# sbyrnes321/metalens

Hardware: AMD Instinct MI355X
Metric: aperture x far-field pair-evals/sec (higher is better)
Workload: dtype f64; 1 GPU; 1 mm dia NA=0.5 lens, lambda=580 nm, 4096x4096 aperture window at pitch lambda/2.2 -> 512x512 far-field directions (bins of the aperture FFT lattice x 1), fp64, on-axis x-dipole at the focus; aperture=4096, farfield=512, rings=197, centre_cells=1219855, orders=survey, pmc_key=gpus=1,aperture=4096,farfield=512,precision=f64,method=auto,zoom=1,pols=1, pmc_stale=True

## Files before the change

metalens_amd/csrc/zfft.hip:

```cpp
#include <cmath>
#include <cstdlib>
#include <map>
#include <tuple>
#include <utility>

#include "common.h"
#include "zfft_core.h"

namespace ml {

using zf::cd;

struct FftArgs {
    zf::Geo g;
    const cd *in;
    int64_t in_s1, in_s2, in_es;
    int in_rb;
    int a0, h0, a1, h1;
    const int *row_first;
    int rf_mod;
    int sub_s, sub_i;
    cd *out;
    int64_t out_s1, out_s2, out_es;
    int out_rb;
    const cd *tw1;
    const cd *wk;
    const cd *pj;
    const int *kbin;
    double alpha[4];
    int alpha_rb;
    int rows, chunk, accumulate;
};

template <int R3T>
__device__ __forceinline__ zf::Geo geo_of(const FftArgs &a) {
    zf::Geo g = a.g;
    if (R3T > 0) g.R3 = R3T;
    return g;
}

template <int R3T, bool STREAM>
__device__ __forceinline__ void load_row(const FftArgs &a, const zf::Geo &g, int row, int tid, cd *v) {
    const int NT = 16 * g.R3;
    const cd *src = a.in + (row / a.in_rb) * a.in_s1 + (row % a.in_rb) * a.in_s2;
    const int first = a.row_first ? a.row_first[row % a.rf_mod] : 0;
#pragma unroll
    for (int n2 = 0; n2 < 16; ++n2) {
        const int n = (tid + NT * n2) * a.sub_s + a.sub_i;
        int q = -1;
        if (n >= a.a0 && n < a.a0 + a.h0) q = n - a.a0;
        if (n >= a.a1 && n < a.a1 + a.h1) q = a.h0 + n - a.a1;
        if (min(n, g.n_valid - 1 - n) < first) q = -1;
        if (STREAM && q >= 0) {
            typedef double double2v __attribute__((ext_vector_type(2)));
            const double2v t = __builtin_nontemporal_load(reinterpret_cast<const double2v *>(src + q * a.in_es));
            v[n2] = zf::mk(t.x, t.y);
        } else {
            v[n2] = q >= 0 ? src[q * a.in_es] : zf::mk(0.0, 0.0);
        }
    }
}

template <int PASS>
__device__ __forceinline__ int64_t out_off(const FftArgs &a, int j) {
    return PASS == 4 ? zf::tile_off(j, a.out_es) : (int64_t)j * a.out_es;
}

__device__ __forceinline__ int row_of_turn(const FftArgs &a, int xcd, int idx) {
    const int row = xcd * a.chunk + idx;
    return idx < a.chunk && row < a.rows ? row : -1;
}

template <int R3T, int NTMAX, int MINW, int PASS, bool IP>
__global__ __launch_bounds__(NTMAX, MINW) void zfft_kernel(const FftArgs a) {
    extern __shared__ __align__(16) unsigned char zfft_lds_raw[];
    cd *lds = reinterpret_cast<cd *>(zfft_lds_raw);
    const zf::Geo g = geo_of<R3T>(a);
    const int NT = 16 * g.R3, tid = threadIdx.x;
    cd *s_tw = lds + zf::lds_elems(g);
    for (int e = tid; e < 256; e += NT) s_tw[(e & 15) * 16 + (e >> 4)] = a.tw1[e];
    const int n1 = tid / g.R3;
    cd tb[4];
    tb[0] = zf::mk(1.0, 0.0);
#pragma unroll
    for (int b = 1; b < 4; ++b) tb[b] = a.tw1[n1 * 16 + b];
    const int bin0 = tid, bin1 = tid + NT;
    const bool own0 = bin0 < g.M, own1 = bin1 < g.M, few = g.M <= 2 * NT;
    cd w0 = zf::mk(0, 0), p0 = w0, w1 = w0, p1 = w0;
    int k0 = 0, k1 = 0;
    if (own0) {
        w0 = a.wk[bin0];
        p0 = a.pj[bin0];
        k0 = a.kbin[bin0];
    }
    if (own1) {
        w1 = a.wk[bin1];
        p1 = a.pj[bin1];
        k1 = a.kbin[bin1];
    }
    const bool pair = own0 && own1 && ((k1 - k0) & 255) == 0;
    __syncthreads();
    const int xcd = blockIdx.x & 7, step = gridDim.x >> 3;
    int idx = blockIdx.x >> 3;
    int row = row_of_turn(a, xcd, idx);
    cd v[16], nx[16];
    if (row >= 0) load_row<R3T, PASS != 2>(a, g, row, tid, v);
    while (row >= 0) {
        const int idx_n = idx + step, row_n = row_of_turn(a, xcd, idx_n);
        const bool more = row_n >= 0;
        if (more) load_row<R3T, PASS != 2>(a, g, row_n, tid, nx);
        {
            cd ta[4];
            ta[0] = tb[0];
#pragma unroll
            for (int q = 1; q < 4; ++q) ta[q] = s_tw[(4 * q) * 16 + n1];
            zf::stage1_regs(g, tid, v, ta, tb, lds);
        }
        __syncthreads();
        zf::gather2(g, tid, v, lds);
        if (IP) {
            zf::scatter2_ip(g, tid, v, lds);
        } else {
            __syncthreads();
            zf::scatter2(g, tid, v, lds);
        }
        __syncthreads();
        cd *dst = a.out + (row / a.out_rb) * a.out_s1 + (row % a.out_rb) * a.out_s2;
        const double al = a.alpha[row / a.alpha_rb];
        if (few && pair) {
            cd xa, xb;
            if (IP)
                zf::stage3_pair_ip(g, k0, w0, w1, lds, xa, xb);
            else
                zf::stage3_pair(g, k0, w0, w1, lds, xa, xb);
            xa = zf::cmul(xa, p0);
            xb = zf::cmul(xb, p1);
            xa.x *= al;
            xa.y *= al;
            xb.x *= al;
            xb.y *= al;
            cd *da = dst + out_off<PASS>(a, bin0), *db = dst + out_off<PASS>(a, bin1);
            if (a.accumulate) {
                xa = zf::cadd(xa, *da);
                xb = zf::cadd(xb, *db);
            }
            *da = xa;
            *db = xb;
        } else if (few) {
            if (own0) {
                cd x = zf::cmul(IP ? zf::stage3_ip(g, k0, w0, lds) : zf::stage3(g, k0, w0, lds), p0);
                x.x *= al;
                x.y *= al;
                cd *d = dst + out_off<PASS>(a, bin0);
                if (a.accumulate) x = zf::cadd(x, *d);
                *d = x;
            }
            if (own1) {
                cd x = zf::cmul(IP ? zf::stage3_ip(g, k1, w1, lds) : zf::stage3(g, k1, w1, lds), p1);
                x.x *= al;
                x.y *= al;
                cd *d = dst + out_off<PASS>(a, bin1);
                if (a.accumulate) x = zf::cadd(x, *d);
                *d = x;
            }
        } else {
            for (int o = tid; o < g.M; o += NT) {
                const cd w = a.wk[o], p = a.pj[o];
                cd x = zf::cmul(IP ? zf::stage3_ip(g, a.kbin[o], w, lds) : zf::stage3(g, a.kbin[o], w, lds), p);
                x.x *= al;
                x.y *= al;
                cd *d = dst + out_off<PASS>(a, o);
                if (a.accumulate) x = zf::cadd(x, *d);
                *d = x;
            }
        }
        __syncthreads();
#pragma unroll
        for (int n2 = 0; n2 < 16; ++n2) v[n2] = nx[n2];
        idx = idx_n;
        row = row_n;
    }
}

template <int A, bool STREAM>
__device__ __forceinline__ void load_row_mixed(const FftArgs &a, const zf::Geo &g, int row, int tid, int stride, cd *v) {
    const cd *src = a.in + (row / a.in_rb) * a.in_s1 + (row % a.in_rb) * a.in_s2;
    const int first = a.row_first ? a.row_first[row % a.rf_mod] : 0;
#pragma unroll
    for (int n2 = 0; n2 < A; ++n2) {
        const int n = tid + stride * n2;
        int q = -1;
        if (n >= a.a0 && n < a.a0 + a.h0) q = n - a.a0;
        if (n >= a.a1 && n < a.a1 + a.h1) q = a.h0 + n - a.a1;
        if (min(n, g.n_valid - 1 - n) < first) q = -1;
        if (STREAM && q >= 0) {
            typedef double double2v __attribute__((ext_vector_type(2)));
            const double2v t = __builtin_nontemporal_load(reinterpret_cast<const double2v *>(src + q * a.in_es));
            v[n2] = zf::mk(t.x, t.y);
        } else {
            v[n2] = q >= 0 ? src[q * a.in_es] : zf::mk(0.0, 0.0);
        }
    }
}

template <int A, int B, bool STREAM>
__global__ __launch_bounds__(512) void zfft_mixed_kernel(const FftArgs a) {
    extern __shared__ __align__(16) unsigned char zfft_lds_raw[];
    cd *lds = reinterpret_cast<cd *>(zfft_lds_raw);
    const zf::Geo g = a.g;
    constexpr int LMAX = A > B ? A : B;
    const int R = g.R3, NT = LMAX * R, tid = threadIdx.x;
    cd *s_tw = lds + zf::mx_lds_elems<A, B>(g);
    for (int e = tid; e < A * B; e += NT) s_tw[(e % A) * B + e / A] = a.tw1[e];
    const bool act1 = tid < B * R, act2 = tid < A * R;
    __syncthreads();
    const int xcd = blockIdx.x & 7, step = gridDim.x >> 3;
    int idx = blockIdx.x >> 3;
    int row = row_of_turn(a, xcd, idx);
    cd v[LMAX], nx[A];
    if (row >= 0 && act1) load_row_mixed<A, STREAM>(a, g, row, tid, B * R, v);
    while (row >= 0) {
        const int idx_n = idx + step, row_n = row_of_turn(a, xcd, idx_n);
        if (row_n >= 0 && act1) load_row_mixed<A, STREAM>(a, g, row_n, tid, B * R, nx);
        if (act1) zf::mx_stage1<A, B>(g, tid, v, s_tw, lds);
        __syncthreads();
        if (act2) zf::mx_stage2<A, B>(g, tid, v, lds);
        __syncthreads();
        cd *dst = a.out + (row / a.out_rb) * a.out_s1 + (row % a.out_rb) * a.out_s2;
        const double al = a.alpha[row / a.alpha_rb];
        for (int o = tid; o < g.M; o += NT) {
            cd x = zf::cmul(zf::mx_stage3<A, B>(g, a.kbin[o], a.wk[o], lds), a.pj[o]);
            x.x *= al;
            x.y *= al;
            cd *d = dst + (int64_t)o * a.out_es;
            if (a.accumulate) x = zf::cadd(x, *d);
            *d = x;
        }
        __syncthreads();
#pragma unroll
        for (int n2 = 0; n2 < A; ++n2) v[n2] = nx[n2];
        idx = idx_n;
        row = row_n;
    }
}

template <int A, int B, bool STREAM>
static int launch_mixed(hipStream_t stream, const FftArgs &a, int threads, int grid, size_t lds_bytes) {
    auto kern = zfft_mixed_kernel<A, B, STREAM>;
    static bool attr_done = false;
    if (!attr_done) {
        ML_HIP(hipFuncSetAttribute(reinterpret_cast<const void *>(kern),
                                   hipFuncAttributeMaxDynamicSharedMemorySize, 160 * 1024));
        attr_done = true;
    }
    hipLaunchKernelGGL(kern, dim3(grid), dim3(threads), lds_bytes, stream, a);
    ML_HIP(hipGetLastError());
    return ML_OK;
}

__device__ __forceinline__ void load_tile(const FftArgs &a, const cd *src, int n0, int m1, cd *v) {
#pragma unroll
    for (int m2 = 0; m2 < 16; ++m2) {
        const int n = n0 + a.g.R3 * (m1 + 16 * m2);
        int q = -1;
        if (n0 >= 0 && n >= a.a0 && n < a.a0 + a.h0) q = n - a.a0;
        if (n0 >= 0 && n >= a.a1 && n < a.a1 + a.h1) q = a.h0 + n - a.a1;
        if (q >= 0) {
            typedef double double2v __attribute__((ext_vector_type(2)));
// ... 127 lines not shown
#pragma unroll
            for (int q = 0; q < (PAIR ? NB / 2 : NB); ++q) {
                const int oa = tid + NT * q, ob = oa + 256;
                if (PAIR) {
                    if (ob < gp.M) {
                        const cd wa = a.wk[oa], wb = a.wk[ob];
                        cd xa, xb;
                        zf::stage3_pair(gp, kq[q], wa, wb, lds, xa, xb);
                        if (p == P - 1) {
                            acc[q] = xa;
                            acc[q + NB / 2] = xb;
                        } else {
                            acc[q] = zf::cmac(acc[q], s_wr[oa], xa);
                            acc[q + NB / 2] = zf::cmac(acc[q + NB / 2], s_wr[ob], xb);
                        }
                        continue;
                    }
                }
                if (oa < gp.M) {
                    const cd wa = a.wk[oa];
                    const cd xa = zf::stage3(gp, kq[q], wa, lds);
                    if (p == P - 1) {
                        acc[q] = xa;
                    } else {
                        acc[q] = zf::cmac(acc[q], s_wr[oa], xa);
                    }
                }
                if (PAIR) acc[q + NB / 2] = zf::mk(0.0, 0.0);
            }
            __syncthreads();
        }
        cd *dst = a.out + (row / a.out_rb) * a.out_s1 + (row % a.out_rb) * a.out_s2;
        const double al = a.alpha[row / a.alpha_rb];
#pragma unroll
        for (int q = 0; q < NB; ++q) {
            const int o = tid + NT * q;
            if (o < gp.M) {
                cd x = zf::cmul(acc[q], a.pj[o]);
                x.x *= al;
                x.y *= al;
                cd *d = dst + o * a.out_es;
                if (a.accumulate) x = zf::cadd(x, *d);
                *d = x;
            }
        }
        idx = idx_n;
        row = row_n;
    }
}

template <int R3P, int P, int NB, int MINW, int PASS>
static int launch_pass(hipStream_t stream, const FftArgs &a, int grid, size_t lds_bytes) {
    auto kern = zfft_pass_kernel<R3P, P, NB, MINW, PASS>;
    static bool attr_done = false;
    if (!attr_done) {
        ML_HIP(hipFuncSetAttribute(reinterpret_cast<const void *>(kern),
                                   hipFuncAttributeMaxDynamicSharedMemorySize, 160 * 1024));
        attr_done = true;
    }
    hipLaunchKernelGGL(kern, dim3(grid), dim3(16 * R3P), lds_bytes, stream, a);
    ML_HIP(hipGetLastError());
    return ML_OK;
}

template <int PASS>
__global__ __launch_bounds__(256) void zfft_multi_kernel(const FftArgs a, int cpw) {
    extern __shared__ __align__(16) unsigned char zfft_lds_raw[];
    const zf::Geo g = a.g;
    const int NT = 16 * g.R3, sub = threadIdx.x / NT, tid = threadIdx.x - sub * NT;
    cd *lds = reinterpret_cast<cd *>(zfft_lds_raw) + (size_t)sub * zf::lds_elems(g);
    cd *s_tw = reinterpret_cast<cd *>(zfft_lds_raw) + (size_t)cpw * zf::lds_elems(g);
    for (int e = threadIdx.x; e < 256; e += blockDim.x) s_tw[(e & 15) * 16 + (e >> 4)] = a.tw1[e];
    const int n1 = tid / g.R3;
    __syncthreads();
    const int groups = (a.rows + cpw - 1) / cpw, chunk = (groups + 7) / 8;
    const int xcd = blockIdx.x & 7, step = gridDim.x >> 3;
    for (int idx = blockIdx.x >> 3; idx < chunk; idx += step) {
        const int grp = xcd * chunk + idx;
        if (grp >= groups) break;
        const int row = grp * cpw + sub;
        const bool live = row < a.rows;
        cd v[16];
        if (live) {
            load_row<0, PASS != 2>(a, g, row, tid, v);
        } else {
#pragma unroll
            for (int n2 = 0; n2 < 16; ++n2) v[n2] = zf::mk(0.0, 0.0);
        }
        zf::stage1_inplace(g, tid, v, s_tw, n1, lds);
        __syncthreads();
        zf::gather2(g, tid, v, lds);
        __syncthreads();
        zf::scatter2(g, tid, v, lds);
        __syncthreads();
        if (live) {
            cd *dst = a.out + (row / a.out_rb) * a.out_s1 + (row % a.out_rb) * a.out_s2;
            const double al = a.alpha[row / a.alpha_rb];
            for (int o = tid; o < g.M; o += NT) {
                cd x = zf::cmul(zf::stage3(g, a.kbin[o], a.wk[o], lds), a.pj[o]);
                x.x *= al;
                x.y *= al;
                cd *d = dst + o * a.out_es;
                if (a.accumulate) x = zf::cadd(x, *d);
                *d = x;
            }
        }
        __syncthreads();
    }
}

__global__ __launch_bounds__(512) void zfft_interleaved_kernel(const FftArgs a, int s, int64_t sub_off, int stuff) {
    extern __shared__ __align__(16) unsigned char zfft_lds_raw[];
    const zf::Geo g = a.g;
    const int NT = 16 * g.R3, sub = threadIdx.x / NT, tid = threadIdx.x - sub * NT, T = NT * s;
    cd *base = reinterpret_cast<cd *>(zfft_lds_raw);
    const int stride = zf::lds_elems(g);
    cd *lds = base + (size_t)sub * stride;
    cd *s_tw = base + (size_t)s * stride;
    for (int e = threadIdx.x; e < 256; e += T) s_tw[(e & 15) * 16 + (e >> 4)] = a.tw1[e];
    const int n1 = tid / g.R3;
    __syncthreads();
    const int chunk = (a.rows + 7) / 8, xcd = blockIdx.x & 7, step = gridDim.x >> 3;
    for (int idx = blockIdx.x >> 3; idx < chunk; idx += step) {
        const int row = xcd * chunk + idx;
        if (row >= a.rows) break;
        const cd *src = a.in + (row / a.in_rb) * a.in_s1 + (row % a.in_rb) * a.in_s2 + sub * sub_off;
        cd v[16];
#pragma unroll
        for (int n2 = 0; n2 < 16; ++n2) {
            const int n = tid + NT * n2, m = n / stuff;
            const int lrow = m * s + sub;
            v[n2] = (m * stuff == n && m < g.n_valid && lrow >= a.a0 && lrow < a.a0 + a.h0) ? src[(int64_t)m * a.in_es]
                                                                                             : zf::mk(0.0, 0.0);
        }
        zf::stage1_inplace(g, tid, v, s_tw, n1, lds);
        __syncthreads();
        zf::gather2(g, tid, v, lds);
        __syncthreads();
        zf::scatter2(g, tid, v, lds);
        __syncthreads();
        cd *dst = a.out + (row / a.out_rb) * a.out_s1 + (row % a.out_rb) * a.out_s2;
        const double al = a.alpha[row / a.alpha_rb];
        for (int o = threadIdx.x; o < g.M; o += T) {
            const int k = a.kbin[o];
            const cd w = a.wk[o];
            cd x = zf::mk(0.0, 0.0);
            for (int i = 0; i < s; ++i)
                x = zf::cmac(zf::stage3(g, k, w, base + (size_t)i * stride), a.pj[(size_t)i * g.M + o], x);
            x.x *= al;
            x.y *= al;
            cd *d = dst + o * a.out_es;
            if (a.accumulate) x = zf::cadd(x, *d);
            *d = x;
        }
        __syncthreads();
    }
}

constexpr int C128_PITCH = 9;
__global__ __launch_bounds__(64) void zfft_cols128_kernel(const FftArgs a, int64_t sub_off) {
    __shared__ cd s_a[8 * 16 * C128_PITCH];
    __shared__ cd s_tw[8 * 16];
    const int lane = threadIdx.x, i = lane >> 3, t = lane & 7;
    for (int e = lane; e < 128; e += 64) s_tw[e] = a.tw1[(2 * (e >> 4)) * 16 + (e & 15)];
    const int M = a.g.M, n_have = a.g.n_valid;
    const int chunk = (a.rows + 7) / 8, xcd = blockIdx.x & 7, step = gridDim.x >> 3;
    for (int idx = blockIdx.x >> 3; idx < chunk; idx += step) {
// ... 243 lines not shown
    }
    const int tiles = c.rows / 8, grid = std::min(tiles, 256);
    hipLaunchKernelGGL(zfft_tiles_kernel, dim3(grid), dim3(L.threads), bytes, stream, a);
    ML_HIP(hipGetLastError());
    return ML_OK;
}

static int zfft_run_mixed(hipStream_t stream, const ZfftCall &c) {
    FftArgs a = args_of(c);
    const int A = c.mixA, B = c.mixB, R = c.N_eff / (A * B), threads = std::max(A, B) * R;
    ML_REQUIRE(A * B * R == c.N_eff && R >= 1 && R <= 32 && threads <= 512 && c.sub_s <= 1 && !c.tiled_out &&
                   c.passes <= 1 && c.pad1 >= 0 && c.pad1 <= 16,
               "mixed-radix transform: %d samples as %d x %d x %d", c.N_eff, A, B, R);
    a.g.R3 = R;
    a.g.pad2 = 0;
    const size_t lds_bytes = ((size_t)(B * R + c.pad1) * A + A * B) * sizeof(cd);
    ML_REQUIRE(lds_bytes <= 160 * 1024, "mixed-radix transform: %d samples do not fit one workgroup", c.N_eff);
    const int per_cu = (int)std::min<size_t>({(size_t)8, std::max<size_t>(1, (160 * 1024) / lds_bytes),
                                              (size_t)std::max(1, 1024 / ((threads + 63) / 64 * 64))});
    int grid = std::min(256 * per_cu, a.chunk * 8);
    grid = (grid + 7) / 8 * 8;
#define ML_MIXED(AA, BB)                                                                            \
    if (A == AA && B == BB)                                                                         \
        return c.in_es == 1 ? launch_mixed<AA, BB, true>(stream, a, threads, grid, lds_bytes)       \
                            : launch_mixed<AA, BB, false>(stream, a, threads, grid, lds_bytes);
    ZF_MX_PAIRS(ML_MIXED)
#undef ML_MIXED
    set_error("mixed-radix transform: no kernel for legs %d x %d", A, B);
    return ML_EINVAL;
}

int zfft_run(hipStream_t stream, const ZfftCall &c) {
    if (c.mixA) return zfft_run_mixed(stream, c);
    FftArgs a = args_of(c);
    ML_REQUIRE(!c.tiled_out || (a.g.R3 >= 3 && a.g.R3 <= 16 && c.passes <= 1 && c.in_es == 1 && !c.second),
               "tiled row pass: %d samples", c.N_eff);
    ZfftLaunchFacts f;
    f.N_eff = c.N_eff, f.M = c.M, f.passes = c.passes;
    f.contiguous = c.in_es == 1, f.second = c.second != 0, f.tiled_out = c.tiled_out != 0;
    const ZfftLaunch L = zfft_launch_rule(f);
    if (L.family == ZfftFamily::multi) {
        const int cpw = L.cpw;
        const size_t bytes = ((size_t)cpw * zf::lds_elems(a.g) + 256) * sizeof(cd);
        const int groups = (a.rows + cpw - 1) / cpw;
        int grid = std::min(256 * 8, (groups + 7) / 8 * 8);
        grid = std::max(grid, 8);
        if (L.PASS == 1)
            hipLaunchKernelGGL(zfft_multi_kernel<1>, dim3(grid), dim3(L.threads), bytes, stream, a, cpw);
        else
            hipLaunchKernelGGL(zfft_multi_kernel<2>, dim3(grid), dim3(L.threads), bytes, stream, a, cpw);
        ML_HIP(hipGetLastError());
        return ML_OK;
    }
    size_t lds_bytes = ((size_t)zf::lds_elems(a.g) + 256) * sizeof(cd);
    const int per_cu = (int)std::min<size_t>(8, std::max<size_t>(1, (160 * 1024) / lds_bytes));
    int grid = std::min(256 * per_cu, a.chunk * 8);
    grid = (grid + 7) / 8 * 8;
    if (L.family == ZfftFamily::pass) {
        const int P = L.P, M = a.g.M;
        FftArgs ap = a;
        zfft_choose_pads(c.N_eff / P, M, c.j0, &ap.g.pad1, &ap.g.pad2, c.jstep);
        zf::Geo gp = ap.g;
        gp.R3 = L.R3P;
        const size_t bytes = ((size_t)zf::lds_elems(gp) + 256 + M) * sizeof(cd);
        const int per = (int)std::min<size_t>(8, std::max<size_t>(1, (160 * 1024) / bytes));
        int gridp = std::min(256 * per, a.chunk * 8);
        gridp = (gridp + 7) / 8 * 8;
#define ML_PASS(R, PP, NBB)                                                                          \
    if (L.R3P == R && L.P == PP && L.NB == NBB)                                                      \
        return L.PASS == 3   ? launch_pass<R, PP, NBB, 2, 3>(stream, ap, gridp, bytes)               \
               : L.PASS == 1 ? launch_pass<R, PP, NBB, 2, 1>(stream, ap, gridp, bytes)               \
                             : launch_pass<R, PP, NBB, 2, 2>(stream, ap, gridp, bytes);
        ML_PASS(16, 2, 2)
        ML_PASS(32, 2, 2)
#undef ML_PASS
    }
    ML_REQUIRE(L.family == ZfftFamily::one, "a lattice of %d samples does not fit one workgroup (%d wanted bins)",
               c.N_eff, c.M);
    if (L.ip) {
        a.g.ip = 1;
        zfft_choose_pads(-c.N_eff, c.M, c.j0, &a.g.pad1, &a.g.pad2, c.jstep);
        lds_bytes = ((size_t)zf::lds_elems(a.g) + 256) * sizeof(cd);
    }
    if (L.PASS == 3) switch (L.R3T) {
            case 8: return launch_one<8, 128, 2, 3>(stream, a, grid, lds_bytes);
            case 16: return launch_one<16, 256, 2, 3>(stream, a, grid, lds_bytes);
            default: return launch_one<32, 512, 2, 3>(stream, a, grid, lds_bytes);
        }
    if (L.PASS == 4) switch (L.R3T) {
            case 4: return launch_one<4, 64, 2, 4>(stream, a, grid, lds_bytes);
            case 8: return launch_one<8, 128, 2, 4>(stream, a, grid, lds_bytes);
            case 16: return launch_one<16, 256, 2, 4>(stream, a, grid, lds_bytes);
            default: return launch_one<0, 512, 1, 4>(stream, a, grid, lds_bytes);
        }
    if (L.PASS == 1) switch (L.R3T) {
            case 4: return launch_one<4, 64, 2, 1>(stream, a, grid, lds_bytes);
            case 8: return launch_one<8, 128, 2, 1>(stream, a, grid, lds_bytes);
            case 16: return launch_one<16, 256, 2, 1>(stream, a, grid, lds_bytes);
            case 32: return launch_one<32, 512, 2, 1>(stream, a, grid, lds_bytes);
            default: return launch_one<0, 512, 1, 1>(stream, a, grid, lds_bytes);
        }
    switch (L.R3T) {
        case 4: return launch_one<4, 64, 2, 2>(stream, a, grid, lds_bytes);
        case 8: return launch_one<8, 128, 2, 2>(stream, a, grid, lds_bytes);
        case 16: return launch_one<16, 256, 2, 2>(stream, a, grid, lds_bytes);
        case 32: return launch_one<32, 512, 2, 2>(stream, a, grid, lds_bytes);
        default: return launch_one<0, 512, 1, 2>(stream, a, grid, lds_bytes);
    }
}

int zfft_choose_pad_mixed(int A, int B, int R, int M, int j0, int jstep) {
    static std::map<std::tuple<int, int, int, int, int, int>, int> memo;
    const auto key = std::make_tuple(A, B, R, M, j0, jstep);
    auto hit = memo.find(key);
    if (hit == memo.end()) {
        zf::Geo g{R, A * B * R, M, j0, 0, 0, 0, jstep};
#define ML_MIXED(AA, BB) \
    if (A == AA && B == BB) zf::mixed_choose_pad<AA, BB>(g);
        ZF_MX_PAIRS(ML_MIXED)
#undef ML_MIXED
        if (memo.size() > 4096) memo.clear();
        hit = memo.emplace(key, g.pad1).first;
    }
    return hit->second;
}

void zfft_choose_pads(int N_eff, int M, int j0, int *pad1, int *pad2, int jstep) {
    static std::map<std::tuple<int, int, int, int>, std::pair<int, int>> memo;
    const auto key = std::make_tuple(N_eff, M, j0, jstep);
    auto hit = memo.find(key);
    if (hit == memo.end()) {
        zf::Geo g{std::abs(N_eff) / 256, std::abs(N_eff), M, j0, 0, 0, N_eff < 0 ? 1 : 0, jstep};
        zf::choose_pads(g);
        if (memo.size() > 4096) memo.clear();
        hit = memo.emplace(key, std::make_pair(g.pad1, g.pad2)).first;
    }
    *pad1 = hit->second.first;
    *pad2 = hit->second.second;
}

}
```

metalens_amd/csrc/zfft_core.h:

```cpp
#pragma once
#include <stdint.h>

#ifdef __HIPCC__
#define ZF_HD __host__ __device__ __forceinline__
#else
#define ZF_HD inline
#include <cmath>
#endif

namespace zf {

struct alignas(16) cd {
    double x, y;
};

ZF_HD cd mk(double x, double y) {
    cd r;
    r.x = x;
    r.y = y;
    return r;
}
ZF_HD cd cadd(cd a, cd b) { return mk(a.x + b.x, a.y + b.y); }
ZF_HD cd csub(cd a, cd b) { return mk(a.x - b.x, a.y - b.y); }
ZF_HD cd cmul(cd a, cd b) {
    return mk(fma(a.x, b.x, -(a.y * b.y)), fma(a.x, b.y, a.y * b.x));
}
ZF_HD cd cmac(cd a, cd b, cd c) {
    return mk(fma(a.x, b.x, fma(-a.y, b.y, c.x)), fma(a.x, b.y, fma(a.y, b.x, c.y)));
}
ZF_HD cd mul_mi(cd a) { return mk(a.y, -a.x); }

ZF_HD void dft4(cd &a, cd &b, cd &c, cd &d) {
    const cd t0 = cadd(a, c), t1 = csub(a, c), t2 = cadd(b, d), t3 = mul_mi(csub(b, d));
    a = cadd(t0, t2);
    c = csub(t0, t2);
    b = cadd(t1, t3);
    d = csub(t1, t3);
}

constexpr double C1 = 0.92387953251128673848;
constexpr double S1 = 0.38268343236508978178;
constexpr double RH = 0.70710678118654757274;

ZF_HD void dft16(cd *v) {
#pragma unroll
    for (int a = 0; a < 4; ++a) dft4(v[a], v[a + 4], v[a + 8], v[a + 12]);
    v[1 + 4] = cmul(v[1 + 4], mk(C1, -S1));
    v[1 + 8] = mk((v[1 + 8].x + v[1 + 8].y) * RH, (v[1 + 8].y - v[1 + 8].x) * RH);
    v[1 + 12] = cmul(v[1 + 12], mk(S1, -C1));
    v[2 + 4] = mk((v[2 + 4].x + v[2 + 4].y) * RH, (v[2 + 4].y - v[2 + 4].x) * RH);
    v[2 + 8] = mul_mi(v[2 + 8]);
    v[2 + 12] = mk((v[2 + 12].y - v[2 + 12].x) * RH, -(v[2 + 12].x + v[2 + 12].y) * RH);
    v[3 + 4] = cmul(v[3 + 4], mk(S1, -C1));
    v[3 + 8] = mk((v[3 + 8].y - v[3 + 8].x) * RH, -(v[3 + 8].x + v[3 + 8].y) * RH);
    v[3 + 12] = cmul(v[3 + 12], mk(-C1, S1));
#pragma unroll
    for (int d = 0; d < 4; ++d) dft4(v[4 * d], v[4 * d + 1], v[4 * d + 2], v[4 * d + 3]);
}
ZF_HD constexpr int bin16(int k) { return (k >> 2) + 4 * (k & 3); }

ZF_HD void dft8(cd *v) {
    cd e0 = v[0], e1 = v[2], e2 = v[4], e3 = v[6], o0 = v[1], o1 = v[3], o2 = v[5], o3 = v[7];
    dft4(e0, e1, e2, e3);
    dft4(o0, o1, o2, o3);
    o1 = mk((o1.x + o1.y) * RH, (o1.y - o1.x) * RH);
    o2 = mul_mi(o2);
    o3 = mk((o3.y - o3.x) * RH, -(o3.x + o3.y) * RH);
    v[0] = cadd(e0, o0);
    v[4] = csub(e0, o0);
    v[1] = cadd(e1, o1);
    v[5] = csub(e1, o1);
    v[2] = cadd(e2, o2);
    v[6] = csub(e2, o2);
    v[3] = cadd(e3, o3);
    v[7] = csub(e3, o3);
}

struct Geo {
    int R3;
    int n_valid;
    int M;
    int j0;
    int pad1;
    int pad2;
    int ip;
    int jstep = 1;
};
ZF_HD int lds_elems(const Geo &g) {
    const int e1 = (16 * g.R3 + g.pad1) * 16, e2 = (256 + g.pad2) * g.R3;
    return (g.ip || e1 > e2) ? e1 : e2;
}
ZF_HD int ex1_addr(const Geo &g, int t, int k2) { return t + (16 * g.R3 + g.pad1) * k2; }
ZF_HD int ex2_addr(const Geo &g, int n0, int k1, int k2) { return k2 + 16 * k1 + (256 + g.pad2) * n0; }
ZF_HD int ex2ip_addr(const Geo &g, int n0, int k1, int k2) { return ex1_addr(g, n0 + g.R3 * k1, k2); }
ZF_HD int bin_of(const Geo &g, int j) {
    const int N = 256 * g.R3;
    long long k = ((long long)(j + g.j0) * g.jstep) % N;
    return (int)(k < 0 ? k + N : k);
}

ZF_HD void stage1_regs(const Geo &g, int t, cd *v, const cd *ta, const cd *tb, cd *lds) {
    dft16(v);
#pragma unroll
    for (int k2 = 0; k2 < 16; ++k2) {
        const int hi = k2 >> 2, lo = k2 & 3;
        cd a = v[bin16(k2)];
        if (hi && lo)
            a = cmul(a, cmul(ta[hi], tb[lo]));
        else if (hi)
            a = cmul(a, ta[hi]);
        else if (lo)
            a = cmul(a, tb[lo]);
        lds[ex1_addr(g, t, k2)] = a;
    }
}
ZF_HD void stage1_inplace(const Geo &g, int t, cd *v, const cd *tw, int n1, cd *lds) {
    dft16(v);
#pragma unroll
    for (int lo = 1; lo < 4; ++lo) {
        const cd w = tw[lo * 16 + n1];
#pragma unroll
        for (int hi = 0; hi < 4; ++hi) v[bin16(4 * hi + lo)] = cmul(v[bin16(4 * hi + lo)], w);
    }
#pragma unroll
    for (int hi = 1; hi < 4; ++hi) {
        const cd w = tw[(4 * hi) * 16 + n1];
#pragma unroll
        for (int lo = 0; lo < 4; ++lo) v[bin16(4 * hi + lo)] = cmul(v[bin16(4 * hi + lo)], w);
    }
#pragma unroll
    for (int k2 = 0; k2 < 16; ++k2) lds[ex1_addr(g, t, k2)] = v[bin16(k2)];
}
ZF_HD void gather2(const Geo &g, int u, cd *v, const cd *lds) {
    const int n0 = u % g.R3, k2 = u / g.R3;
#pragma unroll
    for (int n1 = 0; n1 < 16; ++n1) v[n1] = lds[ex1_addr(g, n0 + g.R3 * n1, k2)];
    dft16(v);
}
ZF_HD void scatter2(const Geo &g, int u, const cd *v, cd *lds) {
    const int n0 = u % g.R3, k2 = u / g.R3;
#pragma unroll
    for (int k1 = 0; k1 < 16; ++k1) lds[ex2_addr(g, n0, k1, k2)] = v[bin16(k1)];
}
ZF_HD void scatter2_ip(const Geo &g, int u, const cd *v, cd *lds) {
    const int n0 = u % g.R3, k2 = u / g.R3;
#pragma unroll
    for (int k1 = 0; k1 < 16; ++k1) lds[ex2ip_addr(g, n0, k1, k2)] = v[bin16(k1)];
}
ZF_HD cd stage3_ip(const Geo &g, int k, cd w, const cd *lds) {
    const cd *b = lds + ex2ip_addr(g, 0, (k >> 4) & 15, k & 15);
    cd x = b[g.R3 - 1];
    for (int n0 = g.R3 - 2; n0 >= 0; --n0) x = cmac(x, w, b[n0]);
    return x;
}
ZF_HD void stage3_pair_ip(const Geo &g, int k, cd wa, cd wb, const cd *lds, cd &xa, cd &xb) {
    const cd *b = lds + ex2ip_addr(g, 0, (k >> 4) & 15, k & 15);
    xa = xb = b[g.R3 - 1];
    for (int n0 = g.R3 - 2; n0 >= 0; --n0) {
        const cd t = b[n0];
        xa = cmac(xa, wa, t);
        xb = cmac(xb, wb, t);
    }
}
ZF_HD cd stage3(const Geo &g, int k, cd w, const cd *lds) {
    const int k2 = k & 15, k1 = (k >> 4) & 15;
    cd x = lds[ex2_addr(g, g.R3 - 1, k1, k2)];
    for (int n0 = g.R3 - 2; n0 >= 0; --n0) x = cmac(x, w, lds[ex2_addr(g, n0, k1, k2)]);
    return x;
}

ZF_HD void stage3_pair(const Geo &g, int k, cd wa, cd wb, const cd *lds, cd &xa, cd &xb) {
    const int k2 = k & 15, k1 = (k >> 4) & 15;
    xa = xb = lds[ex2_addr(g, g.R3 - 1, k1, k2)];
    for (int n0 = g.R3 - 2; n0 >= 0; --n0) {
        const cd t = lds[ex2_addr(g, n0, k1, k2)];
        xa = cmac(xa, wa, t);
        xb = cmac(xb, wb, t);
    }
}

ZF_HD long long tile_off(int j, long long tile) { return (long long)(j >> 3) * tile + (j & 7); }
// ... 127 lines not shown
}
template <int L>
ZF_HD void dft_leg(cd *v) {
    if constexpr (L == 16) {
        dft16(v);
        cd t[16];
#pragma unroll
        for (int k = 0; k < 16; ++k) t[k] = v[bin16(k)];
#pragma unroll
        for (int k = 0; k < 16; ++k) v[k] = t[k];
    } else if constexpr (L == 9) {
        dft_ct<3, 3>(v);
    } else if constexpr (L == 10) {
        dft_ct<5, 2>(v);
    } else if constexpr (L == 12) {
        dft_ct<4, 3>(v);
    } else {
        static_assert(L == 15, "no leg of this size");
        dft_ct<5, 3>(v);
    }
}

template <int A, int B>
ZF_HD int mx_threads(const Geo &g) { return (A > B ? A : B) * g.R3; }
template <int A, int B>
ZF_HD int mx_addr(const Geo &g, int t, int k2) { return t + (B * g.R3 + g.pad1) * k2; }
template <int A, int B>
ZF_HD int mx_lds_elems(const Geo &g) { return (B * g.R3 + g.pad1) * A; }
template <int A, int B>
ZF_HD int mx_bin_of(const Geo &g, int j) {
    const int N = A * B * g.R3;
    long long k = ((long long)(j + g.j0) * g.jstep) % N;
    return (int)(k < 0 ? k + N : k);
}
template <int A, int B>
ZF_HD void mx_stage1(const Geo &g, int t, cd *v, const cd *tw, cd *lds) {
    const int n1 = t / g.R3;
    dft_leg<A>(v);
    lds[mx_addr<A, B>(g, t, 0)] = v[0];
#pragma unroll
    for (int k2 = 1; k2 < A; ++k2) lds[mx_addr<A, B>(g, t, k2)] = cmul(v[k2], tw[k2 * B + n1]);
}
template <int A, int B>
ZF_HD void mx_stage2(const Geo &g, int u, cd *v, cd *lds) {
    const int k2 = u / g.R3, n0 = u - k2 * g.R3;
#pragma unroll
    for (int n1 = 0; n1 < B; ++n1) v[n1] = lds[mx_addr<A, B>(g, n0 + g.R3 * n1, k2)];
    dft_leg<B>(v);
#pragma unroll
    for (int k1 = 0; k1 < B; ++k1) lds[mx_addr<A, B>(g, n0 + g.R3 * k1, k2)] = v[k1];
}
template <int A, int B>
ZF_HD cd mx_stage3(const Geo &g, int k, cd w, const cd *lds) {
    const cd *b = lds + mx_addr<A, B>(g, g.R3 * ((k / A) % B), k % A);
    cd x = b[g.R3 - 1];
    for (int n0 = g.R3 - 2; n0 >= 0; --n0) x = cmac(x, w, b[n0]);
    return x;
}

#define ZF_MX_PAIRS(X) X(16, 15) X(15, 15) X(16, 10) X(15, 10) X(10, 10) X(12, 9) X(9, 9) X(16, 9)
struct MixChoice {
    int s = 0, A = 0, B = 0, R = 0;
};
ZF_HD MixChoice mixed_choose(int N, int M) {
    MixChoice best;
    long long best_cost = -1;
#define ZF_MX_TRY(AA, BB)                                                                              \
    for (int s = 1; s <= 2; ++s) {                                                                     \
        const long long Ne = (long long)N * s;                                                         \
        if (N < 1 || Ne > 8192 || Ne % (AA * BB)) continue;                                            \
        const int R = (int)(Ne / (AA * BB)), NT = (AA > BB ? AA : BB) * R;                             \
        if (R < 1 || R > 32) continue;                                                                 \
        const long long waves = (NT + 63) / 64, cost = waves * (3 * (AA + BB) + (long long)((M + NT - 1) / NT) * R); \
        if (best_cost < 0 || cost < best_cost) {                                                       \
            best_cost = cost;                                                                          \
            best.s = s, best.A = AA, best.B = BB, best.R = R;                                          \
        }                                                                                              \
    }
    ZF_MX_PAIRS(ZF_MX_TRY)
#undef ZF_MX_TRY
    return best;
}

}

namespace zf {

inline int lds_cycles(const int *addr, bool is_read) {
    static const int rd_groups[4][16] = {
        {0, 1, 2, 3, 12, 13, 14, 15, 20, 21, 22, 23, 24, 25, 26, 27},
        {4, 5, 6, 7, 8, 9, 10, 11, 16, 17, 18, 19, 28, 29, 30, 31},
        {32, 33, 34, 35, 44, 45, 46, 47, 52, 53, 54, 55, 56, 57, 58, 59},
        {36, 37, 38, 39, 40, 41, 42, 43, 48, 49, 50, 51, 60, 61, 62, 63}};
    int total = 0;
    const int n_groups = is_read ? 4 : 8, per = is_read ? 16 : 8, slots = is_read ? 16 : 8;
    for (int gidx = 0; gidx < n_groups; ++gidx) {
        int worst = 1;
        for (int s = 0; s < slots; ++s) {
            int seen[16], n_seen = 0;
            for (int q = 0; q < per; ++q) {
                const int lane = is_read ? rd_groups[gidx][q] : gidx * 8 + q;
                const int a = addr[lane];
                if (a < 0 || a % slots != s) continue;
                bool dup = false;
                for (int z = 0; z < n_seen; ++z) dup |= (seen[z] == a);
                if (!dup) seen[n_seen++] = a;
            }
            if (n_seen > worst) worst = n_seen;
        }
        total += worst;
    }
    return total;
}

struct LdsCost {
    long ex1_write = 0, ex1_read = 0, ex2_write = 0, ex2_read = 0, ideal_rw = 0;
};
inline LdsCost lds_cost(const Geo &g) {
    LdsCost c;
    const int NT = 16 * g.R3;
    int addr[64];
    for (int w0 = 0; w0 < NT; w0 += 64) {
        for (int s = 0; s < 16; ++s) {
            for (int l = 0; l < 64; ++l) addr[l] = w0 + l < NT ? ex1_addr(g, w0 + l, s) : -1;
            c.ex1_write += lds_cycles(addr, false);
            for (int l = 0; l < 64; ++l) {
                const int u = w0 + l;
                addr[l] = u < NT ? ex1_addr(g, u % g.R3 + g.R3 * s, u / g.R3) : -1;
            }
            c.ex1_read += lds_cycles(addr, true);
            for (int l = 0; l < 64; ++l) {
                const int u = w0 + l;
                addr[l] = u >= NT ? -1 : g.ip ? ex2ip_addr(g, u % g.R3, s, u / g.R3) : ex2_addr(g, u % g.R3, s, u / g.R3);
            }
            c.ex2_write += lds_cycles(addr, false);
            c.ideal_rw += 4 + 8;
        }
    }
    for (int o0 = 0; o0 < g.M; o0 += 64)
        for (int n0 = 0; n0 < g.R3; ++n0) {
            for (int l = 0; l < 64; ++l) {
                if (o0 + l >= g.M) {
                    addr[l] = -1;
                    continue;
                }
                const int k = bin_of(g, o0 + l);
                addr[l] = g.ip ? ex2ip_addr(g, n0, (k >> 4) & 15, k & 15) : ex2_addr(g, n0, (k >> 4) & 15, k & 15);
            }
            c.ex2_read += lds_cycles(addr, true);
        }
    return c;
}

inline void choose_pads(Geo &g) {
    long best = -1;
    int b1 = 0, b2 = 0;
    for (int p1 = 0; p1 <= 16; ++p1) {
        Geo t = g;
        t.pad1 = p1;
        t.pad2 = 0;
        const LdsCost c = lds_cost(t);
        const long cost = (c.ex1_write + c.ex1_read + (g.ip ? c.ex2_write + c.ex2_read : 0)) * 64 + p1;
        if (best < 0 || cost < best) {
            best = cost;
            b1 = p1;
        }
// ... 95 lines not shown
```

Before: 9262000 billion pair-evals/s.

## Load FFT rows via bounded buffer loads and double-buffer row sets

Adds a buffer-resource row loader that relies on hardware out-of-range zeroing to replace the per-element bounds and windowing checks when the input is a single contiguous run. The main row loop is unrolled by two so that the current and prefetch register sets swap roles instead of copying sixteen complex values per row, with asm barriers marking when loads have arrived. An optional nontemporal tile store is added but disabled by default. This aims to cut load-address arithmetic and register-copy overhead, at the cost of higher register pressure and extra code size.

```diff
diff --git a/metalens_amd/csrc/zfft.hip b/metalens_amd/csrc/zfft.hip
--- a/metalens_amd/csrc/zfft.hip
+++ b/metalens_amd/csrc/zfft.hip
@@ -6,6 +6,13 @@
 
 #include "common.h"
 #include "zfft_core.h"
+
+#ifndef ML_ZFFT_UNROLL2
+#define ML_ZFFT_UNROLL2 1
+#endif
+#ifndef ML_ZFFT_NT_TILES
+#define ML_ZFFT_NT_TILES 0
+#endif
 
 namespace ml {
 
@@ -39,9 +46,36 @@
     return g;
 }
 
-template <int R3T, bool STREAM>
+__device__ __forceinline__ bool one_run(const FftArgs &a) { return a.h1 == 0 && a.in_es == 1; }
+
+template <int COUNT>
+__device__ __forceinline__ void load_row_window(const FftArgs &a, int n_valid, int row, int tid, int stride, int sub_s,
+                                                int sub_i, cd *v) {
+    typedef unsigned int uint4v __attribute__((ext_vector_type(4)));
+    const cd *src = a.in + (row / a.in_rb) * a.in_s1 + (row % a.in_rb) * a.in_s2;
+    const int first = __builtin_amdgcn_readfirstlane(a.row_first ? a.row_first[row % a.rf_mod] : 0);
+    const zf::RowWindow w = zf::row_window(first, n_valid, a.a0, a.h0, sub_s, stride);
+    const uint64_t p = reinterpret_cast<uint64_t>(src + (w.lo - a.a0));
+    const uint64_t pu = (uint64_t)(uint32_t)__builtin_amdgcn_readfirstlane((int)(uint32_t)p) |
+                        ((uint64_t)(uint32_t)__builtin_amdgcn_readfirstlane((int)(uint32_t)(p >> 32)) << 32);
+    const auto rs = __builtin_amdgcn_make_buffer_rsrc(reinterpret_cast<void *>(pu), 0,
+                                                      __builtin_amdgcn_readfirstlane(w.bytes), 0x00020000);
+    const uint32_t base = zf::row_window_base(w, tid, sub_s, sub_i), step = (uint32_t)w.step;
+#pragma unroll
+    for (int n2 = 0; n2 < COUNT; ++n2) {
+        const uint4v t = __builtin_amdgcn_raw_buffer_load_b128(rs, (int)(base + step * (uint32_t)n2), 0, 2);
+        v[n2] = __builtin_bit_cast(cd, t);
+    }
+}
+
+template <int R3T, bool STREAM, bool WINDOW = true>
 __device__ __forceinline__ void load_row(const FftArgs &a, const zf::Geo &g, int row, int tid, cd *v) {
     const int NT = 16 * g.R3;
+    if (STREAM && WINDOW && one_run(a)) {
+        load_row_window<16>(a, g.n_valid, row, tid, NT, a.sub_s, a.sub_i, v);
+        return;
+    }
+    if (STREAM && WINDOW) asm volatile("" : "+v"(tid));
     const cd *src = a.in + (row / a.in_rb) * a.in_s1 + (row % a.in_rb) * a.in_s2;
     const int first = a.row_first ? a.row_first[row % a.rf_mod] : 0;
 #pragma unroll
@@ -71,6 +105,25 @@
     return idx < a.chunk && row < a.rows ? row : -1;
 }
 
+__device__ __forceinline__ void arrived(const cd *v) {
+#pragma unroll
+    for (int i = 0; i < 16; i += 4)
+        asm volatile("" ::"v"(v[i].x), "v"(v[i].y), "v"(v[i + 1].x), "v"(v[i + 1].y), "v"(v[i + 2].x), "v"(v[i + 2].y),
+                     "v"(v[i + 3].x), "v"(v[i + 3].y));
+}
+
+template <int PASS>
+__device__ __forceinline__ void store_bin(cd *d, cd x) {
+    if (PASS == 4 && ML_ZFFT_NT_TILES) {
+        typedef double double2v __attribute__((ext_vector_type(2)));
+        double2v t;
+        t.x = x.x, t.y = x.y;
+        __builtin_nontemporal_store(t, reinterpret_cast<double2v *>(d));
+    } else {
+        *d = x;
+    }
+}
+
 template <int R3T, int NTMAX, int MINW, int PASS, bool IP>
 __global__ __launch_bounds__(NTMAX, MINW) void zfft_kernel(const FftArgs a) {
     extern __shared__ __align__(16) unsigned char zfft_lds_raw[];
@@ -103,87 +156,108 @@
     const int xcd = blockIdx.x & 7, step = gridDim.x >> 3;
     int idx = blockIdx.x >> 3;
     int row = row_of_turn(a, xcd, idx);
+    constexpr int SETS = ML_ZFFT_UNROLL2 && PASS != 2 ? 2 : 1;
     cd v[16], nx[16];
-    if (row >= 0) load_row<R3T, PASS != 2>(a, g, row, tid, v);
+    if (SETS == 2) {
+#pragma unroll
+        for (int n2 = 0; n2 < 16; ++n2) nx[n2] = zf::mk(0.0, 0.0);
+    }
+    if (row >= 0) {
+        load_row<R3T, PASS != 2>(a, g, row, tid, v);
+        if (SETS == 2) arrived(v);
+    }
     while (row >= 0) {
-        const int idx_n = idx + step, row_n = row_of_turn(a, xcd, idx_n);
-        const bool more = row_n >= 0;
-        if (more) load_row<R3T, PASS != 2>(a, g, row_n, tid, nx);
-        {
-            cd ta[4];
-            ta[0] = tb[0];
-#pragma unroll
-            for (int q = 1; q < 4; ++q) ta[q] = s_tw[(4 * q) * 16 + n1];
-            zf::stage1_regs(g, tid, v, ta, tb, lds);
-        }
-        __syncthreads();
-        zf::gather2(g, tid, v, lds);
-        if (IP) {
-            zf::scatter2_ip(g, tid, v, lds);
-        } else {
+#pragma unroll
+        for (int h = 0; h < SETS; ++h) {
+            cd *cur = h ? nx : v, *ahead = h ? v : nx;
+            const int idx_n = idx + step, row_n = row_of_turn(a, xcd, idx_n);
+            const bool more = row_n >= 0;
+            if (more) load_row<R3T, PASS != 2>(a, g, row_n, tid, ahead);
+            {
+                cd ta[4];
+                ta[0] = tb[0];
+    #pragma unroll
+                for (int q = 1; q < 4; ++q) ta[q] = s_tw[(4 * q) * 16 + n1];
+                zf::stage1_regs(g, tid, cur, ta, tb, lds);
+            }
             __syncthreads();
-            zf::scatter2(g, tid, v, lds);
-        }
-        __syncthreads();
-        cd *dst = a.out + (row / a.out_rb) * a.out_s1 + (row % a.out_rb) * a.out_s2;
-        const double al = a.alpha[row / a.alpha_rb];
-        if (few && pair) {
-            cd xa, xb;
-            if (IP)
-                zf::stage3_pair_ip(g, k0, w0, w1, lds, xa, xb);
-            else
-                zf::stage3_pair(g, k0, w0, w1, lds, xa, xb);
-            xa = zf::cmul(xa, p0);
-            xb = zf::cmul(xb, p1);
-            xa.x *= al;
-            xa.y *= al;
-            xb.x *= al;
-            xb.y *= al;
-            cd *da = dst + out_off<PASS>(a, bin0), *db = dst + out_off<PASS>(a, bin1);
-            if (a.accumulate) {
-                xa = zf::cadd(xa, *da);
-                xb = zf::cadd(xb, *db);
-            }
-            *da = xa;
-            *db = xb;
-        } else if (few) {
-            if (own0) {
-                cd x = zf::cmul(IP ? zf::stage3_ip(g, k0, w0, lds) : zf::stage3(g, k0, w0, lds), p0);
-                x.x *= al;
-                x.y *= al;
-                cd *d = dst + out_off<PASS>(a, bin0);
-                if (a.accumulate) x = zf::cadd(x, *d);
-                *d = x;
-            }
-            if (own1) {
-                cd x = zf::cmul(IP ? zf::stage3_ip(g, k1, w1, lds) : zf::stage3(g, k1, w1, lds), p1);
-                x.x *= al;
-                x.y *= al;
-                cd *d = dst + out_off<PASS>(a, bin1);
-                if (a.accumulate) x = zf::cadd(x, *d);
-                *d = x;
-            }
-        } else {
-            for (int o = tid; o < g.M; o += NT) {
-                const cd w = a.wk[o], p = a.pj[o];
-                cd x = zf::cmul(IP ? zf::stage3_ip(g, a.kbin[o], w, lds) : zf::stage3(g, a.kbin[o], w, lds), p);
-                x.x *= al;
-                x.y *= al;
-                cd *d = dst + out_off<PASS>(a, o);
-                if (a.accumulate) x = zf::cadd(x, *d);
-                *d = x;
-            }
-        }
-        __syncthreads();
-#pragma unroll
-        for (int n2 = 0; n2 < 16; ++n2) v[n2] = nx[n2];
-        idx = idx_n;
-        row = row_n;
+            zf::gather2(g, tid, cur, lds);
+            if (IP) {
+                zf::scatter2_ip(g, tid, cur, lds);
+            } else {
+                __syncthreads();
+                zf::scatter2(g, tid, cur, lds);
+            }
+            __syncthreads();
+            cd *dst = a.out + (row / a.out_rb) * a.out_s1 + (row % a.out_rb) * a.out_s2;
+            const double al = a.alpha[row / a.alpha_rb];
+            if (few && pair) {
+                cd xa, xb;
+                if (IP)
+                    zf::stage3_pair_ip(g, k0, w0, w1, lds, xa, xb);
+                else
+                    zf::stage3_pair(g, k0, w0, w1, lds, xa, xb);
+                xa = zf::cmul(xa, p0);
+                xb = zf::cmul(xb, p1);
+                xa.x *= al;
+                xa.y *= al;
+                xb.x *= al;
+                xb.y *= al;
+                cd *da = dst + out_off<PASS>(a, bin0), *db = dst + out_off<PASS>(a, bin1);
+                if (a.accumulate) {
+                    xa = zf::cadd(xa, *da);
+                    xb = zf::cadd(xb, *db);
+                }
+                store_bin<PASS>(da, xa);
+                store_bin<PASS>(db, xb);
+            } else if (few) {
+                if (own0) {
+                    cd x = zf::cmul(IP ? zf::stage3_ip(g, k0, w0, lds) : zf::stage3(g, k0, w0, lds), p0);
+                    x.x *= al;
+                    x.y *= al;
+                    cd *d = dst + out_off<PASS>(a, bin0);
+                    if (a.accumulate) x = zf::cadd(x, *d);
+                    store_bin<PASS>(d, x);
+                }
+                if (own1) {
+                    cd x = zf::cmul(IP ? zf::stage3_ip(g, k1, w1, lds) : zf::stage3(g, k1, w1, lds), p1);
+                    x.x *= al;
+                    x.y *= al;
+                    cd *d = dst + out_off<PASS>(a, bin1);
+                    if (a.accumulate) x = zf::cadd(x, *d);
+                    store_bin<PASS>(d, x);
+                }
+            } else {
+                for (int o = tid; o < g.M; o += NT) {
+                    const cd w = a.wk[o], p = a.pj[o];
+                    cd x = zf::cmul(IP ? zf::stage3_ip(g, a.kbin[o], w, lds) : zf::stage3(g, a.kbin[o], w, lds), p);
+                    x.x *= al;
+                    x.y *= al;
+                    cd *d = dst + out_off<PASS>(a, o);
+                    if (a.accumulate) x = zf::cadd(x, *d);
+                    store_bin<PASS>(d, x);
+                }
+            }
+            __syncthreads();
+            if (SETS == 1) {
+#pragma unroll
+                for (int n2 = 0; n2 < 16; ++n2) v[n2] = nx[n2];
+            } else {
+                arrived(ahead);
+            }
+            idx = idx_n;
+            row = row_n;
+            if (SETS == 2 && !more) break;
+        }
     }
 }
 
 template <int A, bool STREAM>
 __device__ __forceinline__ void load_row_mixed(const FftArgs &a, const zf::Geo &g, int row, int tid, int stride, cd *v) {
+    if (STREAM && one_run(a)) {
+        load_row_window<A>(a, g.n_valid, row, tid, stride, 1, 0, v);
+        return;
+    }
     const cd *src = a.in + (row / a.in_rb) * a.in_s1 + (row % a.in_rb) * a.in_s2;
     const int first = a.row_first ? a.row_first[row % a.rf_mod] : 0;
 #pragma unroll
@@ -477,7 +551,7 @@
         const bool live = row < a.rows;
         cd v[16];
         if (live) {
-            load_row<0, PASS != 2>(a, g, row, tid, v);
+            load_row<0, PASS != 2, false>(a, g, row, tid, v);
         } else {
 #pragma unroll
             for (int n2 = 0; n2 < 16; ++n2) v[n2] = zf::mk(0.0, 0.0);
diff --git a/metalens_amd/csrc/zfft_core.h b/metalens_amd/csrc/zfft_core.h
--- a/metalens_amd/csrc/zfft_core.h
+++ b/metalens_amd/csrc/zfft_core.h
@@ -97,6 +97,23 @@
     const int N = 256 * g.R3;
     long long k = ((long long)(j + g.j0) * g.jstep) % N;
     return (int)(k < 0 ? k + N : k);
+}
+
+struct RowWindow {
+    int lo;
+    int bytes;
+    int step;
+};
+ZF_HD RowWindow row_window(int first, int n_valid, int a0, int h0, int sub_s, int NT) {
+    const int lo = a0 > first ? a0 : first, hi = a0 + h0 < n_valid - first ? a0 + h0 : n_valid - first;
+    RowWindow w;
+    w.lo = hi > lo ? lo : a0;
+    w.bytes = hi > lo ? 16 * (hi - lo) : 0;
+    w.step = 16 * NT * sub_s;
+    return w;
+}
+ZF_HD uint32_t row_window_base(const RowWindow &w, int tid, int sub_s, int sub_i) {
+    return (uint32_t)(16 * (tid * sub_s + sub_i - w.lo));
 }
 
 ZF_HD void stage1_regs(const Geo &g, int t, cd *v, const cd *ta, const cd *tb, cd *lds) {
```

Result: no change. 9336000 billion pair-evals/s (median of 6 runs) (+0.8%).

## Add specialized fixed-shape row FFT kernel with software-pipelined row loads

Applied to the files above, without the earlier changes.

Adds a dedicated persistent-row kernel for the in-place single-workgroup FFT path when the bin count equals twice the thread count and inputs are unit-strided. Each workgroup walks its rows with incremental divide-free index walkers, double-buffers the next row's nontemporal global loads in registers while the current row's LDS stages run, and stages twiddles in LDS once per block. The goal is to hide global load latency and cut per-row index arithmetic and generic-path overhead. The cost is a second code path with hand-placed waitcnt values and tighter applicability conditions, which risks register pressure and correctness fragility.

```diff
diff --git a/metalens_amd/csrc/zfft.hip b/metalens_amd/csrc/zfft.hip
--- a/metalens_amd/csrc/zfft.hip
+++ b/metalens_amd/csrc/zfft.hip
@@ -6,6 +6,7 @@
 
 #include "common.h"
 #include "zfft_core.h"
+#include "zfft_rows.h"
 
 namespace ml {
 
@@ -887,6 +888,19 @@
         zfft_choose_pads(-c.N_eff, c.M, c.j0, &a.g.pad1, &a.g.pad2, c.jstep);
         lds_bytes = ((size_t)zf::lds_elems(a.g) + 256) * sizeof(cd);
     }
+    {
+        static const bool rows_off = [] { const char *e = getenv("METALENS_HIP_FIXED_ROWS"); return e && e[0] == '0'; }();
+        zf::RowsFacts rf;
+        rf.family_one = L.family == ZfftFamily::one, rf.ip = L.ip, rf.PASS = L.PASS, rf.R3 = a.g.R3, rf.M = a.g.M;
+        rf.sub_s = a.sub_s, rf.sub_i = a.sub_i, rf.in_es = a.in_es, rf.accumulate = a.accumulate;
+        rf.a0 = a.a0, rf.h0 = a.h0, rf.a1 = a.a1, rf.h1 = a.h1, rf.n_valid = a.g.n_valid;
+        rf.out_last = L.PASS == 4 ? zf::tile_off(a.g.M - 1, a.out_es) : (int64_t)(a.g.M - 1) * a.out_es;
+        if (!rows_off && zf::rows_kernel_takes(rf)) {
+            static const int rows_grid = [] { const char *e = getenv("METALENS_HIP_FIXED_ROWS_GRID"); return e ? atoi(e) : 0; }();
+            const int g8 = rows_grid > 0 ? std::min(grid, (rows_grid + 7) / 8 * 8) : grid;
+            return zfft_rows_run(stream, c, a.g.pad1, g8, lds_bytes);
+        }
+    }
     if (L.PASS == 3) switch (L.R3T) {
             case 8: return launch_one<8, 128, 2, 3>(stream, a, grid, lds_bytes);
             case 16: return launch_one<16, 256, 2, 3>(stream, a, grid, lds_bytes);
diff --git a/metalens_amd/csrc/zfft_core.h b/metalens_amd/csrc/zfft_core.h
--- a/metalens_amd/csrc/zfft_core.h
+++ b/metalens_amd/csrc/zfft_core.h
@@ -390,6 +390,47 @@
     return best;
 }
 
+ZF_HD void row_run(int first, int n_valid, int &lo, int &hi) {
+    lo = first, hi = n_valid - first;
+    if (hi <= lo) lo = hi = 0;
+}
+ZF_HD bool piece_lane(int n, int lo, int hi) { return (unsigned)(n - lo) < (unsigned)(hi - lo); }
+
+ZF_HD int rows_begin(int block, int chunk) { return (block & 7) * chunk + (block >> 3); }
+ZF_HD int rows_end(int block, int chunk, int rows) {
+    const int e = ((block & 7) + 1) * chunk;
+    return e < rows ? e : rows;
+}
+struct RowWalk {
+    int q, r, d, dq, dr;
+};
+ZF_HD RowWalk walk_init(int row, int d, int step) {
+    RowWalk w;
+    w.q = row / d, w.r = row % d, w.d = d, w.dq = step / d, w.dr = step % d;
+    return w;
+}
+ZF_HD void walk_step(RowWalk &w) {
+    w.q += w.dq;
+    w.r += w.dr;
+    if (w.r >= w.d) w.r -= w.d, ++w.q;
+}
+
+struct RowsFacts {
+    bool family_one = false, ip = false;
+    int PASS = 0, R3 = 0, M = 0;
+    int sub_s = 1, sub_i = 0, a0 = 0, h0 = 0, a1 = 0, h1 = 0, n_valid = 0, accumulate = 0;
+    long long in_es = 1;
+    long long out_last = 0;
+};
+ZF_HD bool rows_kernel_takes(const RowsFacts &f) {
+    if (!f.family_one || !f.ip || (f.PASS != 1 && f.PASS != 4) || (f.R3 != 8 && f.R3 != 16)) return false;
+    if (f.M != 2 * 16 * f.R3) return false;
+    if (f.sub_s != 1 || f.sub_i != 0 || f.in_es != 1) return false;
+    if (f.h1 != 0 || f.a0 != 0 || f.h0 < f.n_valid || f.n_valid < 0 || f.n_valid > 256 * f.R3) return false;
+    if (f.accumulate) return false;
+    return f.out_last >= 0 && f.out_last < (1LL << 27);
+}
+
 }
 
 namespace zf {
diff --git a/metalens_amd/csrc/zfft_rows.h b/metalens_amd/csrc/zfft_rows.h
--- /dev/null
+++ b/metalens_amd/csrc/zfft_rows.h
@@ -0,0 +1,8 @@
+#pragma once
+#include "common.h"
+
+namespace ml {
+
+int zfft_rows_run(hipStream_t stream, const ZfftCall &c, int pad1, int grid, size_t lds_bytes);
+
+}
diff --git a/metalens_amd/csrc/zfft_rows.hip b/metalens_amd/csrc/zfft_rows.hip
--- /dev/null
+++ b/metalens_amd/csrc/zfft_rows.hip
@@ -0,0 +1,192 @@
+#include <type_traits>
+
+#include "zfft_rows.h"
+#include "zfft_core.h"
+
+namespace ml {
+
+using zf::cd;
+
+struct RowsArgs {
+    int n_valid, pad1;
+    const cd *in;
+    int64_t in_s1, in_s2;
+    int in_rb;
+    const int *row_first;
+    int rf_mod;
+    cd *out;
+    int64_t out_s1, out_s2, out_es;
+    int out_rb;
+    const cd *tw1, *wk, *pj;
+    const int *kbin;
+    double alpha[4];
+    int alpha_rb;
+    int rows, chunk;
+};
+
+typedef double double2v __attribute__((ext_vector_type(2)));
+
+__device__ __forceinline__ uint32_t here(uint32_t off) {
+    asm volatile("" : "+v"(off));
+    return off;
+}
+
+template <int NT>
+__device__ __forceinline__ void rows_load(const cd *src, int lo, int hi, int tid, uint32_t lane_off, int pitch, cd *v) {
+    const char *base = reinterpret_cast<const char *>(src);
+    const int rel = tid - lo;
+#pragma unroll
+    for (int n2 = 0; n2 < 16; ++n2) {
+        double2v t = {0.0, 0.0};
+        if (zf::piece_lane(rel + NT * n2, 0, hi - lo))
+            t = __builtin_nontemporal_load(reinterpret_cast<const double2v *>(base + here(lane_off)));
+        v[n2] = zf::mk(t.x, t.y);
+        base += pitch;
+    }
+}
+
+template <int R3T, bool TILED>
+__global__ __launch_bounds__(16 * R3T, 2) void zfft_rows_kernel(const RowsArgs a) {
+    extern __shared__ __align__(16) unsigned char zfft_rows_lds_raw[];
+    cd *lds = reinterpret_cast<cd *>(zfft_rows_lds_raw);
+    constexpr int NT = 16 * R3T;
+    const int tid = threadIdx.x;
+    const int step = gridDim.x >> 3, row_end = zf::rows_end(blockIdx.x, a.chunk, a.rows);
+    int row = zf::rows_begin(blockIdx.x, a.chunk);
+    if (row >= row_end) return;
+    zf::Geo g;
+    g.R3 = R3T, g.n_valid = a.n_valid, g.M = 2 * NT, g.j0 = 0, g.pad1 = a.pad1, g.pad2 = 0, g.ip = 1;
+    cd *s_tw = lds + zf::lds_elems(g);
+    for (int e = tid; e < 256; e += NT) s_tw[(e & 15) * 16 + (e >> 4)] = a.tw1[e];
+    const int n1 = tid / R3T;
+    cd tb[4];
+    tb[0] = zf::mk(1.0, 0.0);
+#pragma unroll
+    for (int b = 1; b < 4; ++b) tb[b] = a.tw1[n1 * 16 + b];
+    const int bin0 = tid, bin1 = tid + NT;
+    const cd w0 = a.wk[bin0], p0 = a.pj[bin0], w1 = a.wk[bin1], p1 = a.pj[bin1];
+    const int k0 = a.kbin[bin0], k1 = a.kbin[bin1];
+    const uint32_t off0 = (uint32_t)((TILED ? zf::tile_off(bin0, a.out_es) : (long long)bin0 * a.out_es) * 16);
+    const uint32_t off1 = (uint32_t)((TILED ? zf::tile_off(bin1, a.out_es) : (long long)bin1 * a.out_es) * 16);
+    const uint32_t lane_off = (uint32_t)tid * 16;
+    int pitch = NT * 16;
+    asm volatile("" : "+s"(pitch));
+    __syncthreads();
+
+    zf::RowWalk wi = zf::walk_init(row, a.in_rb, step), wf = zf::walk_init(row, a.rf_mod, step);
+    zf::RowWalk wo = zf::walk_init(row, a.out_rb, step), wa = zf::walk_init(row, a.alpha_rb, step);
+    typedef const int __attribute__((address_space(4))) * const_int_ptr;
+    const const_int_ptr rf = (const_int_ptr)(uintptr_t)a.row_first;
+    cd va[16], vb[16];
+    int lo, hi;
+    zf::row_run(rf ? rf[wf.r] : 0, a.n_valid, lo, hi);
+    rows_load<NT>(a.in + wi.q * a.in_s1 + wi.r * a.in_s2, lo, hi, tid, lane_off, pitch, va);
+    zf::walk_step(wi);
+    zf::walk_step(wf);
+    int row_n = row + step;
+    int first_n = rf && row_n < row_end ? rf[wf.r] : 0;
+
+    auto turn = [&](auto first_turn, cd *v, cd *nx) __attribute__((always_inline)) -> bool {
+        const bool more = row_n < row_end;
+        if (decltype(first_turn)::value)
+            __builtin_amdgcn_s_waitcnt(0x0f70);
+        else
+            __builtin_amdgcn_s_waitcnt(0x0f72);
+        if (more) {
+            zf::row_run(first_n, a.n_valid, lo, hi);
+            rows_load<NT>(a.in + wi.q * a.in_s1 + wi.r * a.in_s2, lo, hi, tid, lane_off, pitch, nx);
+            zf::walk_step(wi);
+            zf::walk_step(wf);
+            first_n = rf && row_n + step < row_end ? rf[wf.r] : 0;
+        }
+        {
+            cd ta[4];
+            ta[0] = tb[0];
+#pragma unroll
+            for (int q = 1; q < 4; ++q) ta[q] = s_tw[(4 * q) * 16 + n1];
+            zf::stage1_regs(g, tid, v, ta, tb, lds);
+        }
+        __syncthreads();
+        zf::gather2(g, tid, v, lds);
+        zf::scatter2_ip(g, tid, v, lds);
+        __syncthreads();
+        char *dst = reinterpret_cast<char *>(a.out + wo.q * a.out_s1 + wo.r * a.out_s2);
+        const double al = a.alpha[wa.q];
+        cd xa, xb;
+        if (NT % 256 == 0) {
+            zf::stage3_pair_ip(g, k0, w0, w1, lds, xa, xb);
+        } else {
+            xa = zf::stage3_ip(g, k0, w0, lds);
+            xb = zf::stage3_ip(g, k1, w1, lds);
+        }
+        xa = zf::cmul(xa, p0);
+        xb = zf::cmul(xb, p1);
+        xa.x *= al;
+        xa.y *= al;
+        xb.x *= al;
+        xb.y *= al;
+        *reinterpret_cast<cd *>(dst + here(off0)) = xa;
+        *reinterpret_cast<cd *>(dst + here(off1)) = xb;
+        __syncthreads();
+        zf::walk_step(wo);
+        zf::walk_step(wa);
+        row = row_n;
+        row_n += step;
+        return more;
+    };
+    if (turn(std::true_type(), va, vb))
+        for (;;) {
+            if (!turn(std::false_type(), vb, va)) break;
+            if (!turn(std::false_type(), va, vb)) break;
+        }
+}
+
+template <int R3T, bool TILED>
+static int launch_rows(hipStream_t stream, const RowsArgs &a, int grid, size_t lds_bytes) {
+    auto kern = zfft_rows_kernel<R3T, TILED>;
+    static bool attr_done = false;
+    if (!attr_done) {
+        ML_HIP(hipFuncSetAttribute(reinterpret_cast<const void *>(kern), hipFuncAttributeMaxDynamicSharedMemorySize,
+                                   160 * 1024));
+        attr_done = true;
+    }
+    hipLaunchKernelGGL(kern, dim3(grid), dim3(16 * R3T), lds_bytes, stream, a);
+    ML_HIP(hipGetLastError());
+    return ML_OK;
+}
+
+int zfft_rows_run(hipStream_t stream, const ZfftCall &c, int pad1, int grid, size_t lds_bytes) {
+    const int R3 = c.N_eff / 256;
+    ML_REQUIRE((R3 == 8 || R3 == 16) && c.M == 32 * R3 && grid > 0 && grid % 8 == 0 && c.in_rb > 0 && c.out_rb > 0 &&
+                   c.alpha_rb > 0 && c.rows <= 4 * (int64_t)c.alpha_rb,
+               "fixed-shape row transform: %d samples, %d bins, %d rows", c.N_eff, c.M, c.rows);
+    RowsArgs a;
+    a.n_valid = c.n_valid;
+    a.pad1 = pad1;
+    a.in = reinterpret_cast<const cd *>(c.in);
+    a.in_s1 = c.in_s1;
+    a.in_s2 = c.in_s2;
+    a.in_rb = c.in_rb;
+    a.row_first = c.row_first;
+    a.rf_mod = c.rf_mod > 0 ? c.rf_mod : 1;
+    a.out = reinterpret_cast<cd *>(c.out);
+    a.out_s1 = c.out_s1;
+    a.out_s2 = c.out_s2;
+    a.out_es = c.out_es;
+    a.out_rb = c.out_rb;
+    a.tw1 = reinterpret_cast<const cd *>(c.tw1);
+    a.wk = reinterpret_cast<const cd *>(c.wk);
+    a.pj = reinterpret_cast<const cd *>(c.pj);
+    a.kbin = c.kbin;
+    for (int k = 0; k < 4; ++k) a.alpha[k] = c.alpha[k];
+    a.alpha_rb = c.alpha_rb;
+    a.rows = c.rows;
+    a.chunk = (c.rows + 7) / 8;
+    if (R3 == 16)
+        return c.tiled_out ? launch_rows<16, true>(stream, a, grid, lds_bytes)
+                           : launch_rows<16, false>(stream, a, grid, lds_bytes);
+    return c.tiled_out ? launch_rows<8, true>(stream, a, grid, lds_bytes)
+                       : launch_rows<8, false>(stream, a, grid, lds_bytes);
+}
+
+}
```

After: 9574000 billion pair-evals/s before, 9731000 billion pair-evals/s after (median of 6 runs). +1.6%, better.
